# XiaRho/MADM

Measured on AMD Instinct MI355X. Metric: UNet feature-extract images/sec @512x512 bs=2/GPU, higher is better.
Workload: dtype f16; 1 GPU; configs[1]: SD-v1-4 VAE-encode + UNet single-timestep feature extractor (taps 5,8,11 'after'), 2x3x512x512 per GPU, t=0, LoRA off (shipped configs), seeded synthetic weights; global_batch=2, parallelism=replicas x1 (no collectives)

## Files before the change

madm_amd/csrc/conv3x3.hip:

```cpp
#include "conv3x3_common.hpp"

namespace {

template <typename T, int BN, bool FUSE, int NWS>
__global__ __launch_bounds__(256, (NWS == 2 || BN == 64) ? 2 : 1) void conv3x3_halo_kernel(const IgemmP p, const PatchDecode pd) {
    kernarg_touch<5>();
    constexpr int EPC = TT<T>::EPC;
    constexpr int BKE = 8 * EPC;
    constexpr int MI = 4, NI = BN / 32;
    constexpr int RB = BN / 32;
    constexpr int HI = (HPIX * 8 + 255) / 256;
    constexpr int HALO_U4 = HPIX * 8, W_U4 = BN * 8;
    constexpr unsigned OOB = 0x80000000u;
    extern __shared__ __attribute__((aligned(16))) char smem_raw[];
    u32x4* halo = reinterpret_cast<u32x4*>(smem_raw);
    u32x4* wlds = halo + 2 * HALO_U4;
    float2* gstat = reinterpret_cast<float2*>(wlds + 2 * W_U4);

    const int tid = threadIdx.x, lane = tid & 63, wave = tid >> 6;
    const int wm = wave >> 1, wn = wave & 1;
    const int cpos = tid & 7, lrow = tid >> 3;
    const int frow = lane & 15, fg = lane >> 4;
    const int z = blockIdx.z;

// ... 175 lines not shown
        }                                                                                           \
        C3_PRIO(0);                                                                                 \
        C3_PIN();                                                                                   \
        C3_STAMP(s_, 1);                                                                            \
        if ((s_) + 1 < S) C3_STORE_W((CUR) ^ 1, RS_);                                               \
        if (tap == 8 && next_chunk_) C3_STORE_HALO(((ck - ck0) + 1) & 1, ck + 1);                   \
        C3_STAMP(s_, 2);                                                                            \
        __syncthreads();                                                                            \
        C3_STAMP(s_, 3);                                                                            \
        if (++tap == 9) { tap = 0; ++ck; }                                                          \
    }
    int s = 0;
    if constexpr (NWS == 2) {
        for (; s + 1 < S; s += 2) {
            C3_STEP(s, 0, rw[0], rw[1]);
            C3_STEP(s + 1, 1, rw[1], rw[0]);
        }
        if (s < S) C3_STEP(s, 0, rw[0], rw[1]);
    } else {
        for (; s + NWS <= S; s += NWS) {
#pragma unroll
            for (int u = 0; u < NWS; ++u) C3_STEP(s + u, u & 1, rw[u], rw[(u + 1) % NWS]);
        }
#pragma unroll
        for (int u = 0; u < NWS - 1; ++u)
            if (s + u < S) C3_STEP(s + u, u & 1, rw[u], rw[(u + 1) % NWS]);
    }
#undef C3_STEP
#undef C3_LOAD_W
#undef C3_STORE_W
#undef C3_LOAD_HALO
#undef C3_STORE_HALO

    halo_tile_epilogue<T, BN>(p, acc, b, py0, px0, n0, z, reinterpret_cast<float*>(smem_raw));
}

template <typename T, int BN, bool FUSE, int NWS>
int launch_one(const IgemmP& p0, hipStream_t s) {
    IgemmP p = p0;
    constexpr size_t lds = (size_t)(2 * HPIX * 8 + 2 * BN * 8) * 16 + 32 * sizeof(float2);
    auto kern = conv3x3_halo_kernel<T, BN, FUSE, NWS>;
    static std::atomic<uint64_t> attr_done{0};
    if (int e = madm_raise_dynamic_lds(reinterpret_cast<const void*>(kern), (size_t)(lds), attr_done, "conv3x3")) return e;
    const int patchesX = (p.OW + TW - 1) / TW, patchesY = (p.OH + TH - 1) / TH;
    p.tilesN = (p.N + BN - 1) / BN;
    dim3 grid((unsigned)(p.B * patchesX * patchesY * p.tilesN), 1, (unsigned)p.splitk);
    PatchDecode pd;
    if (!patch_decode_fill(pd, patchesX, patchesY, p.tilesN, (long long)grid.x)) {
        madm_set_error("conv3x3: grid of %u blocks too large for the reciprocal patch decode", grid.x);
        return MADM_ERR_INVALID_ARG;
    }
    kern<<<grid, 256, lds, s>>>(p, pd);
    return madm_check_launch("conv3x3_halo_kernel");
}

}

template <typename T>
int launch_conv3x3_halo(const IgemmP& p, int bn, hipStream_t s) {
    const bool fuse = p.gn_sums1 != nullptr;
    if (bn == 128) return fuse ? launch_one<T, 128, true, 2>(p, s) : launch_one<T, 128, false, 2>(p, s);
    return fuse ? launch_one<T, 64, true, 2>(p, s) : launch_one<T, 64, false, 2>(p, s);
}
#ifdef C3_STAMPS
extern "C" int madm_debug_read_c3_stamps(unsigned long long* host, int n) {
    return (int)hipMemcpyFromSymbol(host, HIP_SYMBOL(g_c3_stamps), sizeof(unsigned long long) * n);
}
// ... 5 lines not shown
```

madm_amd/csrc/conv3x3_common.hpp:

```cpp
#pragma once
#include "igemm_common.hpp"

struct PatchDecode {
    int patchesX, patchesPerImg;
    unsigned m_tilesN, m_ppi, m_px;
};
__host__ inline unsigned patch_magic(unsigned d) { return d <= 1 ? 0u : (unsigned)((0x100000000ull + d - 1) / d); }
__host__ inline bool patch_decode_fill(PatchDecode& pd, int patchesX, int patchesY, int tilesN, long long blocks) {
    pd.patchesX = patchesX; pd.patchesPerImg = patchesX * patchesY;
    pd.m_tilesN = patch_magic((unsigned)tilesN); pd.m_ppi = patch_magic((unsigned)pd.patchesPerImg);
    pd.m_px = patch_magic((unsigned)patchesX);
    const unsigned long long lim = 0x100000000ull;
    return (unsigned long long)blocks * (unsigned)tilesN < lim && (unsigned long long)blocks * (unsigned)pd.patchesPerImg < lim &&
           (unsigned long long)pd.patchesPerImg * (unsigned)patchesX < lim;
}
__device__ __forceinline__ int magic_div(int x, unsigned m) { return m ? (int)__umulhi((unsigned)x, m) : x; }

namespace {

constexpr int TH = 8, TW = 16, HWD = TW + 2, HPIX = (TH + 2) * HWD;
#ifdef C3_STAMPS
__device__ unsigned long long g_c3_stamps[2048];
#endif

template <typename T, int EPC>
__device__ __forceinline__ u32x4 gn_act_chunk(u32x4 raw, const float* sc, const float* sh, int act) {
    float f[EPC];
    chunk_to_f32<T>(__builtin_bit_cast(uint4, raw), f);
#pragma unroll
    for (int j = 0; j < EPC; ++j) f[j] = f[j] * sc[j] + sh[j];
    act_inplace<EPC>(f, act);
    return __builtin_bit_cast(u32x4, f32_to_chunk<T>(f));
}

template <typename T, int BN>
__device__ __forceinline__ void halo_tile_epilogue(const IgemmP& p, f32x4 (&acc)[4][BN / 32], int b, int py0, int px0,
                                                   int n0, int z, float* red) {
    constexpr int MI = 4, NI = BN / 32;
    const int tid = threadIdx.x, lane = tid & 63, wave = tid >> 6;
    const int wm = wave >> 1, wn = wave & 1;
    const int frow = lane & 15, fg = lane >> 4;
    const bool want_stats = p.stats != nullptr && p.splitk == 1;
    const int nb = n0 + wn * (BN / 2) + fg * 4;
    f32x4 cs[NI], cq[NI], add[NI];
#pragma unroll
    for (int j = 0; j < NI; ++j) { cs[j] = f32x4{0.f, 0.f, 0.f, 0.f}; cq[j] = f32x4{0.f, 0.f, 0.f, 0.f}; }
    if (p.splitk == 1) epilogue_consts<NI>(p, nb, b, add);
    int mrow[MI];
#pragma unroll
    for (int i = 0; i < MI; ++i) {
        const int oy = py0 + wm * 4 + i, ox = px0 + frow;
        mrow[i] = (oy < p.OH && ox < p.OW) ? (b * p.OH + oy) * p.OW + ox : -1;
    }
    if (p.splitk > 1) {
#pragma unroll
        for (int i = 0; i < MI; ++i) {
            if (mrow[i] < 0) continue;
#pragma unroll
            for (int j = 0; j < NI; ++j) {
                const f32x4 v = acc[i][j];
                if (nb + 16 * j < p.N)
                    *reinterpret_cast<float4*>(p.ws + ((size_t)z * p.M + mrow[i]) * p.N + nb + 16 * j) =
                        make_float4(v[0], v[1], v[2], v[3]);
            }
        }
    } else {
        epilogue_tile<T, MI, NI>(p, mrow, nb, add, false, acc);
        if (want_stats) {
#pragma unroll
            for (int i = 0; i < MI; ++i) {
                if (mrow[i] < 0) continue;
#pragma unroll
                for (int j = 0; j < NI; ++j)
                    if (nb + 16 * j < p.N) { cs[j] += acc[i][j]; cq[j] += acc[i][j] * acc[i][j]; }
            }
        }
    }
    if (want_stats) {
#pragma unroll
        for (int j = 0; j < NI; ++j) {
#pragma unroll
            for (int r = 0; r < 4; ++r) {
                cs[j][r] = row16_sum(cs[j][r]);
                cq[j][r] = row16_sum(cq[j][r]);
            }
            if (frow == 0) {
                float* dst = red + ((wm * BN) + wn * (BN / 2) + j * 16 + fg * 4) * 2;
#pragma unroll
                for (int r = 0; r < 4; ++r) { dst[2 * r] = cs[j][r]; dst[2 * r + 1] = cq[j][r]; }
            }
        }
    }
    if (want_stats) {
        __syncthreads();
        for (int c = tid; c < 2 * BN; c += 256) {
            const int n = n0 + (c >> 1);
            if (n < p.N)
                atomicAdd(p.stats + ((size_t)b * p.N + n0) * 2 + c, (double)red[c] + (double)red[2 * BN + c]);
        }
    }
}

}
```

madm_amd/csrc/conv3x3_dma.hip:

```cpp
#include "conv3x3_common.hpp"

namespace {

#if defined(__HIP_DEVICE_COMPILE__)
template <int N> __device__ __forceinline__ void c3_wait_vmcnt() { asm volatile("s_waitcnt vmcnt(%0)" ::"n"(N) : "memory"); }
template <int N> __device__ __forceinline__ void c3_wait_lgkmcnt() { asm volatile("s_waitcnt lgkmcnt(%0)" ::"n"(N) : "memory"); }
#endif

#ifdef C3D_STAMPS
__device__ unsigned long long g_c3d_stamps[256];
#define C3D_STAMP(k_) if (blockIdx.x == 5 && blockIdx.z == 0 && threadIdx.x == 0 && (k_) < 256) g_c3d_stamps[(k_)] = __builtin_readcyclecounter();
#else
#define C3D_STAMP(k_)
#endif

template <typename T, int BN, bool FUSE>
__global__ __launch_bounds__(256, 2) void conv3x3_halo_dma_kernel(const IgemmP p, const PatchDecode pd) {
    C3D_STAMP(0);
    kernarg_touch<5>();
#if defined(__HIP_DEVICE_COMPILE__)
    constexpr int EPC = TT<T>::EPC;
    constexpr int BKE = 8 * EPC;
    constexpr int MI = 4, NI = BN / 32;
    constexpr int LW = BN / 32;
// ... 180 lines not shown
                for (int i = 0; i < MI; ++i)
                    asm volatile("ds_read_b128 %0, %1" : "=v"(af[1][i]) : "v"(ah[(r_ + i) * 3 + sx_] ^ 64u));
#pragma unroll
                for (int j = 0; j < NI; ++j)
                    asm volatile("ds_read_b128 %0, %1 offset:%2" : "=v"(wf[1][j]) : "v"(wf1), "n"(cur * kW_BYTES + j * 2048));
                c3_wait_lgkmcnt<MI + NI>();
                __builtin_amdgcn_sched_barrier(0);
#pragma unroll
                for (int i = 0; i < MI; ++i)
#pragma unroll
                    for (int j = 0; j < NI; ++j)
                        mma16<T>(__builtin_bit_cast(uint4, wf[0][j]), __builtin_bit_cast(uint4, af[0][i]), acc[i][j]);
                c3_wait_lgkmcnt<0>();
                __builtin_amdgcn_sched_barrier(0);
#pragma unroll
                for (int i = 0; i < MI; ++i)
#pragma unroll
                    for (int j = 0; j < NI; ++j)
                        mma16<T>(__builtin_bit_cast(uint4, wf[1][j]), __builtin_bit_cast(uint4, af[1][i]), acc[i][j]);
            }
            __builtin_amdgcn_sched_barrier(0);
            if (tap == 8 && next_chunk) {
                __builtin_amdgcn_s_barrier();
                D3_STORE_HALO(ck + 1);
            }
        }
    }
#undef D3_LOAD_HALO
#undef D3_STORE_HALO
#undef D3_DMA_W
    C3D_STAMP(4);
    c3_wait_vmcnt<0>();
    __syncthreads();
    halo_tile_epilogue<T, BN>(p, acc, b, py0, px0, n0, z, reinterpret_cast<float*>(smem_raw));
    C3D_STAMP(5);
#ifdef C3D_STAMPS
    asm volatile("s_waitcnt vmcnt(0)" ::: "memory");
    C3D_STAMP(6);
#endif
#endif
}

template <typename T, int BN, bool FUSE>
int launch_dma_one(const IgemmP& p0, hipStream_t s) {
    IgemmP p = p0;
    constexpr size_t lds = (size_t)(HPIX * 8 + 3 * BN * 8) * 16 + 32 * sizeof(float2);
    auto kern = conv3x3_halo_dma_kernel<T, BN, FUSE>;
    static std::atomic<uint64_t> attr_done{0};
    if (int e = madm_raise_dynamic_lds(reinterpret_cast<const void*>(kern), (size_t)(lds), attr_done, "conv3x3 (LDS-DMA)")) return e;
    const int patchesX = (p.OW + TW - 1) / TW, patchesY = (p.OH + TH - 1) / TH;
    p.tilesN = (p.N + BN - 1) / BN;
    dim3 grid((unsigned)(p.B * patchesX * patchesY * p.tilesN), 1, (unsigned)p.splitk);
    PatchDecode pd;
    if (!patch_decode_fill(pd, patchesX, patchesY, p.tilesN, (long long)grid.x)) {
        madm_set_error("conv3x3 (LDS-DMA): grid of %u blocks too large for the reciprocal patch decode", grid.x);
        return MADM_ERR_INVALID_ARG;
    }
    kern<<<grid, 256, lds, s>>>(p, pd);
    return madm_check_launch("conv3x3_halo_dma_kernel");
}

}

template <typename T>
int launch_conv3x3_halo_dma(const IgemmP& p, int bn, hipStream_t s) {
    const bool fuse = p.gn_sums1 != nullptr;
    if (bn == 128) return fuse ? launch_dma_one<T, 128, true>(p, s) : launch_dma_one<T, 128, false>(p, s);
// ... 11 lines not shown
```

madm_amd/csrc/igemm.hip:

```cpp
#include <algorithm>
#include <cstdio>
#include <cstdlib>
#include <vector>
#include <atomic>
#include "igemm_common.hpp"

namespace {
#ifdef GLDS_STAMPS
__device__ unsigned long long g_reg_stamps[64];
#define REG_BSTAMP(k_) if (blockIdx.x == 7 && blockIdx.z == 0 && threadIdx.x == 0) g_reg_stamps[(k_)] = __builtin_readcyclecounter();
#else
#define REG_BSTAMP(k_)
#endif

template <int BM, int BN>
__device__ __forceinline__ bool cstash_request(const IgemmP& p, int m0, int n0, u32x4& cb, u32x4& cr, u32x4& cl) {
    constexpr unsigned OOB = 0x80000000u;
    const int tid = threadIdx.x;
    const bool on = p.splitk == 1 && tid < BN / 4;
    const unsigned nbytes = (unsigned)p.N * 4u;
    const float* rowp = nullptr;
    if (p.rowvec) {
        const int OHW = p.OH * p.OW;
        int mlast = m0 + BM; if (mlast > p.M) mlast = p.M; mlast -= 1;
        const int img0 = m0 / OHW;
        if (mlast / OHW == img0) rowp = p.rowvec + (size_t)img0 * p.ldrv;
    }
    const float* dummy = reinterpret_cast<const float*>(p.w);
    const __amdgpu_buffer_rsrc_t rb = __builtin_amdgcn_make_buffer_rsrc((void*)(p.bias ? p.bias : dummy), 0, p.bias ? nbytes : 0u, 0x00020000);
    const __amdgpu_buffer_rsrc_t rr = __builtin_amdgcn_make_buffer_rsrc((void*)(rowp ? rowp : dummy), 0, rowp ? nbytes : 0u, 0x00020000);
    const __amdgpu_buffer_rsrc_t rl = __builtin_amdgcn_make_buffer_rsrc((void*)(p.ln_cs ? p.ln_cs : dummy), 0, p.ln_cs ? nbytes : 0u, 0x00020000);
    const unsigned off = on ? (unsigned)(n0 + tid * 4) * 4u : OOB;
    cb = __builtin_amdgcn_raw_buffer_load_b128(rb, off, 0, 0);
    cr = __builtin_amdgcn_raw_buffer_load_b128(rr, off, 0, 0);
    cl = __builtin_amdgcn_raw_buffer_load_b128(rl, off, 0, 0);
    return on;
}
template <int BN>
__device__ __forceinline__ void cstash_park(bool on, u32x4 cb_, u32x4 cr_, u32x4 cl_, float* cstash) {
    if (on) {
        const float4 cb = __builtin_bit_cast(float4, cb_), cr = __builtin_bit_cast(float4, cr_);
        *reinterpret_cast<float4*>(cstash + threadIdx.x * 4) = make_float4(cb.x + cr.x, cb.y + cr.y, cb.z + cr.z, cb.w + cr.w);
        *reinterpret_cast<float4*>(cstash + BN + threadIdx.x * 4) = __builtin_bit_cast(float4, cl_);
    }
}

template <typename T, int BM, int BN>
__device__ __forceinline__ void igemm_tile_epilogue(const IgemmP& p, f32x4 (&acc)[BM / 32][BN / 32], int m0, int n0,
                                                    int z, float* red, float (&lns)[BM / 32], float (&lnq)[BM / 32],
                                                    const float* cstash, const float* cstash_row, const float* cstash_ln) {
    constexpr int MI = BM / 32, NI = BN / 32;
    const int tid = threadIdx.x, lane = tid & 63, wave = tid >> 6;
    const int wm = wave >> 1, wn = wave & 1;
    const int frow = lane & 15, fg = lane >> 4;
    const int OHW = p.OH * p.OW;
    const bool want_stats = p.stats != nullptr && p.splitk == 1;
    int mlast = m0 + BM; if (mlast > p.M) mlast = p.M; mlast -= 1;
    const int img0 = m0 / OHW;
    const bool one_image = (mlast / OHW) == img0;
    const int nb = n0 + wn * (BN / 2) + fg * 4;
    f32x4 cs[NI], cq[NI], add[NI];
#pragma unroll
    for (int j = 0; j < NI; ++j) { cs[j] = f32x4{0.f, 0.f, 0.f, 0.f}; cq[j] = f32x4{0.f, 0.f, 0.f, 0.f}; }
    if (p.splitk == 1) {
#pragma unroll
        for (int j = 0; j < NI; ++j) {
            const float4 c = *reinterpret_cast<const float4*>(cstash + wn * (BN / 2) + fg * 4 + 16 * j);
            add[j] = f32x4{c.x, c.y, c.z, c.w};
            if (cstash_row) {
                const float4 r = *reinterpret_cast<const float4*>(cstash_row + wn * (BN / 2) + fg * 4 + 16 * j);
                add[j] += f32x4{r.x, r.y, r.z, r.w};
            }
        }
    }
    if (p.ln_cs) {
        f32x4 csv[NI];
#pragma unroll
        for (int j = 0; j < NI; ++j) {
            const float4 c = *reinterpret_cast<const float4*>(cstash_ln + wn * (BN / 2) + fg * 4 + 16 * j);
            csv[j] = f32x4{c.x, c.y, c.z, c.w};
        }
        const float inv_k = 1.0f / (float)p.K;
        float2* lx = reinterpret_cast<float2*>(red + 4 * BN);
#pragma unroll
        for (int i = 0; i < MI; ++i) {
            float sx = lns[i], sq = lnq[i];
            sx += __shfl_xor(sx, 16); sq += __shfl_xor(sq, 16);
            sx += __shfl_xor(sx, 32); sq += __shfl_xor(sq, 32);
            lns[i] = sx; lnq[i] = sq;
            if (fg == 0) lx[(wave * MI + i) * 16 + frow] = make_float2(sx, sq);
        }
        __syncthreads();
#pragma unroll
        for (int i = 0; i < MI; ++i) {
            const float2 o = lx[((wave ^ 1) * MI + i) * 16 + frow];
            const float sx = lns[i] + o.x, sq = lnq[i] + o.y;
            const float mean = sx * inv_k;
            float var = sq * inv_k - mean * mean;
            var = var < 0.f ? 0.f : var;
            const float rstd = 1.0f / sqrtf(var + p.ln_eps);
#pragma unroll
            for (int j = 0; j < NI; ++j) acc[i][j] = (acc[i][j] - mean * csv[j]) * rstd;
        }
    }
    REG_BSTAMP(8);
    int mrow[MI];
#pragma unroll
    for (int i = 0; i < MI; ++i) {
        const int m = m0 + wm * (BM / 2) + i * 16 + frow;
        mrow[i] = m < p.M ? m : -1;
    }
    if (p.splitk > 1) {
#pragma unroll
        for (int i = 0; i < MI; ++i) {
            if (mrow[i] < 0) continue;
#pragma unroll
            for (int j = 0; j < NI; ++j) {
                const f32x4 v = acc[i][j];
                if (nb + 16 * j < p.N)
                    *reinterpret_cast<float4*>(p.ws + ((size_t)z * p.M + mrow[i]) * p.N + nb + 16 * j) =
                        make_float4(v[0], v[1], v[2], v[3]);
            }
        }
    } else {
        epilogue_tile<T, MI, NI>(p, mrow, nb, add, !one_image, acc);
        if (want_stats) {
#pragma unroll
            for (int i = 0; i < MI; ++i) {
                if (mrow[i] < 0) continue;
#pragma unroll
                for (int j = 0; j < NI; ++j) {
                    if (nb + 16 * j >= p.N) continue;
                    if (one_image) { cs[j] += acc[i][j]; cq[j] += acc[i][j] * acc[i][j]; }
                    else stats_add_elementwise(p, mrow[i], nb + 16 * j, acc[i][j]);
                }
            }
        }
    }
    REG_BSTAMP(9 + MI);
    if (want_stats && one_image) {
#pragma unroll
        for (int j = 0; j < NI; ++j) {
#pragma unroll
            for (int r = 0; r < 4; ++r) {
                cs[j][r] = row16_sum(cs[j][r]);
                cq[j][r] = row16_sum(cq[j][r]);
            }
            if (frow == 0) {
                float* dst = red + ((wm * BN) + wn * (BN / 2) + j * 16 + fg * 4) * 2;
#pragma unroll
                for (int r = 0; r < 4; ++r) { dst[2 * r] = cs[j][r]; dst[2 * r + 1] = cq[j][r]; }
            }
        }
    }
    if (want_stats && one_image) {
        __syncthreads();
        for (int c = tid; c < 2 * BN; c += 256) {
            const int n = n0 + (c >> 1);
            if (n < p.N) atomicAdd(p.stats + ((size_t)img0 * p.N + n0) * 2 + c, (double)red[c] + (double)red[2 * BN + c]);
        }
    }
}

template <typename T, int BM, int BN, int NST, bool LIN>
__global__ __launch_bounds__(256, (BM * BN >= 128 * 128) ? 1 : 2) void igemm_kernel(const IgemmP p) {
    kernarg_touch<5>();
    constexpr int EPC = TT<T>::EPC;
    constexpr int BKE = 8 * EPC;
    constexpr int RA = BM / 32, RB = BN / 32;
    constexpr int MI = BM / 32, NI = BN / 32;
    __shared__ __attribute__((aligned(16))) uint4 smem[2 * (BM + BN) * 8];
    __shared__ __attribute__((aligned(16))) float cstash[2 * BN];

    const int tid = threadIdx.x, lane = tid & 63, wave = tid >> 6;
    REG_BSTAMP(0);
    const int wm = wave >> 1, wn = wave & 1;
    int bid = blockIdx.x;
    {
        const int nb = gridDim.x, q = nb >> 3, r = nb & 7, x = bid & 7, i = bid >> 3;
        bid = (x < r ? x * (q + 1) : r * (q + 1) + (x - r) * q) + i;
    }
    const int tn = bid % p.tilesN, tm = bid / p.tilesN;
    const int m0 = tm * BM, n0 = tn * BN;
    const int z = blockIdx.z;
    const int chunk = tid & 7, lrow = tid >> 3;
// ... 115 lines not shown
            uint4 af[MI], wf[NI];                                                                   \
            _Pragma("unroll") for (int i = 0; i < MI; ++i)                                          \
                af[i] = sA[(wm * (BM / 2) + i * 16 + frow) * 8 + c];                                \
            _Pragma("unroll") for (int j = 0; j < NI; ++j)                                          \
                wf[j] = sB[(wn * (BN / 2) + j * 16 + frow) * 8 + c];                                \
            _Pragma("unroll") for (int i = 0; i < MI; ++i)                                          \
                _Pragma("unroll") for (int j = 0; j < NI; ++j) mma16<T>(wf[j], af[i], acc[i][j]);   \
            if (ln_on && kk == wn) {    \
                _Pragma("unroll") for (int i = 0; i < MI; ++i) ln_accum<T>(af[i], lns[i], lnq[i]);  \
            }                                                                                       \
        }                                                                                           \
    }
    REG_BSTAMP(2);
    for (int kt = kt0; kt < kt1; kt += NST) {
#pragma unroll
        for (int u = 0; u < NST; ++u) {
            const int t = kt + u;
            if (t < kt1) {
                const int cur = (t - kt0) & 1;
                if (t + NST < kt1) IGEMM_LOAD_TILE(t + NST, ra[u], rb[u]);
                __builtin_amdgcn_sched_barrier(0);
                IGEMM_COMPUTE(cur);
                __builtin_amdgcn_sched_barrier(0);
                if (t + 1 < kt1) IGEMM_STORE_TILE(cur ^ 1, ra[(u + 1) % NST], rb[(u + 1) % NST]);
                __syncthreads();
            }
        }
    }
#undef IGEMM_COMPUTE
#undef IGEMM_LOAD_TILE
#undef IGEMM_STORE_TILE

    REG_BSTAMP(3);
    igemm_tile_epilogue<T, BM, BN>(p, acc, m0, n0, z, reinterpret_cast<float*>(smem), lns, lnq, cstash, nullptr, cstash + BN);
    REG_BSTAMP(4);
#ifdef GLDS_STAMPS
    asm volatile("s_waitcnt vmcnt(0)" ::: "memory");
    REG_BSTAMP(5);
#endif
}

#define GLDS_ASM(...) asm volatile(__VA_ARGS__)
#ifdef GLDS_STAMPS
__device__ unsigned long long g_glds_stamps[2048];
#endif
#if defined(__HIP_DEVICE_COMPILE__)
template <int N> __device__ __forceinline__ void wait_vmcnt() { GLDS_ASM("s_waitcnt vmcnt(%0)" ::"n"(N) : "memory"); }
template <int N> __device__ __forceinline__ void wait_lgkmcnt() { GLDS_ASM("s_waitcnt lgkmcnt(%0)" ::"n"(N) : "memory"); }
#endif

template <typename T, int BM, int BN, int NS, bool LIN>
__global__ __launch_bounds__(256, BM * BN >= 128 * 128 ? (NS == 2 ? 2 : 1) : (NS == 3 && BM == 64 ? 3 : 2)) void igemm_glds_kernel(const IgemmP p) {
#if defined(__HIP_DEVICE_COMPILE__)
    kernarg_touch<5>();
    constexpr int EPC = TT<T>::EPC;
    constexpr int BKE = 8 * EPC;
    constexpr int MI = BM / 32, NI = BN / 32;
    constexpr int ROWS = BM + BN;
    constexpr int LPT = ROWS / 32;
    constexpr int TILE_U4 = ROWS * 8;
    static_assert(NS >= 2 && NS <= 4 && ROWS % 32 == 0, "ring depth / tile shape");
    extern __shared__ __attribute__((aligned(16))) uint4 gsmem[];
    __shared__ __attribute__((aligned(16))) float cstash[3 * 256];
    typedef __attribute__((address_space(3))) char lds_char;

    const int tid = threadIdx.x, lane = tid & 63;
    const int wave = __builtin_amdgcn_readfirstlane(tid >> 6);
    const int wm = wave >> 1, wn = wave & 1;
#ifdef GLDS_STAMPS
#define GLDS_BSTAMP(k_) if (blockIdx.x == 0 && blockIdx.z == 0 && tid == 0) g_glds_stamps[2000 + (k_)] = __builtin_readcyclecounter();
#else
#define GLDS_BSTAMP(k_)
#endif
    GLDS_BSTAMP(0);
    int bid = blockIdx.x;
    {
        const int nb = gridDim.x, q = nb >> 3, r = nb & 7, x = bid & 7, i = bid >> 3;
        bid = (x < r ? x * (q + 1) : r * (q + 1) + (x - r) * q) + i;
    }
    const int tn = bid % p.tilesN, tm = bid / p.tilesN;
    const int m0 = tm * BM, n0 = tn * BN;
    const int z = blockIdx.z;
    const int rsub = lane >> 3, cpos = lane & 7;

    constexpr unsigned OOB = 0x80000000u;
    const int OHW = p.OH * p.OW;
    int a_b[LPT], a_iy[LPT], a_ix[LPT];
    unsigned wvoff[LPT], swz[LPT];
#pragma unroll
    for (int i = 0; i < LPT; ++i) {
        const int row = (wave * LPT + i) * 8 + rsub;
        swz[i] = (unsigned)((cpos ^ (row & 7)) * EPC);
        a_b[i] = 0; a_iy[i] = -(1 << 24); a_ix[i] = 0; wvoff[i] = OOB;
        if (row < BM) {
// ... 149 lines not shown
            _Pragma("unroll") for (int i = 0; i < MI; ++i)                                                       \
                _Pragma("unroll") for (int j = 0; j < NI; ++j)                                                   \
                    mma16<T>(__builtin_bit_cast(uint4, wf[0][j]), __builtin_bit_cast(uint4, af[0][i]), acc[i][j]); \
            wait_lgkmcnt<0>();                                                                                   \
            __builtin_amdgcn_sched_barrier(0);                                                                   \
            _Pragma("unroll") for (int i = 0; i < MI; ++i)                                                       \
                _Pragma("unroll") for (int j = 0; j < NI; ++j)                                                   \
                    mma16<T>(__builtin_bit_cast(uint4, wf[1][j]), __builtin_bit_cast(uint4, af[1][i]), acc[i][j]); \
            if (ln_on) {                 \
                if (wn == 0) {                                                                                   \
                    _Pragma("unroll") for (int i = 0; i < MI; ++i)                                               \
                        ln_accum<T>(__builtin_bit_cast(uint4, af[0][i]), lns[i], lnq[i]);                        \
                } else {                                                                                         \
                    _Pragma("unroll") for (int i = 0; i < MI; ++i)                                               \
                        ln_accum<T>(__builtin_bit_cast(uint4, af[1][i]), lns[i], lnq[i]);                        \
                }                                                                                                \
            }                                                                                                    \
        }                                                                                                        \
        __builtin_amdgcn_sched_barrier(0);                                                                       \
        GLDS_STAMP(t, 3);                                                                                        \
    }
    int t = 0;
    for (; t + NS <= nt; t += NS) {
#pragma unroll
        for (int u = 0; u < NS; ++u) GLDS_STEP(t + u, u, (u + NS - 1) % NS);
    }
#pragma unroll
    for (int u = 0; u < NS - 1; ++u)
        if (t + u < nt) GLDS_STEP(t + u, u, (u + NS - 1) % NS);
#undef GLDS_STEP
#undef GLDS_LOAD_TILE
    GLDS_BSTAMP(3);
    __syncthreads();
    igemm_tile_epilogue<T, BM, BN>(p, acc, m0, n0, z, reinterpret_cast<float*>(gsmem), lns, lnq, cstash, cstash + 256, cstash + 512);
    GLDS_BSTAMP(4);
#endif
}

template <typename T>
__global__ __launch_bounds__(256) void splitk_reduce_kernel(const IgemmP p) {
    __shared__ float red[16][64][2];
    const int tx = threadIdx.x & 15, ty = threadIdx.x >> 4;
    const int n = (blockIdx.x * 16 + tx) * 4;
    const int mbase = blockIdx.y * 16;
    const int OHW = p.OH * p.OW;
    int mlast = mbase + 16; if (mlast > p.M) mlast = p.M; mlast -= 1;
    const int img0 = mbase / OHW;
    const bool one_image = (mlast / OHW) == img0;
    const bool want_stats = p.stats != nullptr;
    f32x4 v = f32x4{0.f, 0.f, 0.f, 0.f};
    const int m = mbase + ty;
    const bool valid = m < p.M && n < p.N;
    if (valid) {
        const bool plain = p.epilogue != MADM_EPI_GEGLU;
        f32x4 add = f32x4{0.f, 0.f, 0.f, 0.f}, res = f32x4{0.f, 0.f, 0.f, 0.f};
        if (plain) {
            if (p.bias) {
                const float4 b = *reinterpret_cast<const float4*>(p.bias + n);
                add = f32x4{b.x, b.y, b.z, b.w};
            }
            if (p.rowvec) {
                const float4 r = *reinterpret_cast<const float4*>(p.rowvec + (size_t)(m / OHW) * p.ldrv + n);
                add[0] += r.x; add[1] += r.y; add[2] += r.z; add[3] += r.w;
            }
            if (p.residual) res = load4<T>(reinterpret_cast<const T*>(p.residual) + (size_t)m * p.ldr + n);
        }
        const float* src = p.ws + (size_t)m * p.N + n;
// ... 316 lines not shown
        MADM_REQUIRE(a->KH == 1 && a->KW == 1 && a->stride == 1 && a->pad_t == 0 && a->pad_l == 0 && !a->upsample &&
                     a->C2 == 0 && a->OH == a->IH && a->OW == a->IW,
                     "conv2d: the folded LayerNorm needs a linear layer / 1x1 conv over ONE source (K = C1)");
        MADM_REQUIRE(!a->gn_sums1 && a->ln_eps > 0.f && a->splitk == 1,
                     "conv2d: folded LayerNorm: no fused GroupNorm, eps > 0, splitk == 1 (every block must see whole rows)");
    }
    MADM_REQUIRE(!a->stats || a->epilogue != MADM_EPI_GEGLU, "conv2d: fused statistics cannot follow GEGLU");
    p.C1 = a->C1; p.C2 = a->C2; p.Ctot = a->C1 + a->C2;
    p.B = a->B; p.IH = a->IH; p.IW = a->IW; p.OH = a->OH; p.OW = a->OW;
    p.KH = a->KH; p.KW = a->KW; p.stride = a->stride; p.pad_t = a->pad_t; p.pad_l = a->pad_l;
    p.upsample = a->upsample ? 1 : 0;
    p.N = a->N; p.K = r.K; p.M = r.M;
    MADM_REQUIRE(!a->rowvec || (a->ldrv >= a->N && a->ldrv % 4 == 0), "conv2d: bad ldrv=%d", a->ldrv);
    p.ldr = a->ldr; p.ldo = a->ldo; p.ldrv = a->ldrv; p.epilogue = a->epilogue;
    p.ldw = a->ldw ? a->ldw : p.K;
    p.out_f32 = a->out_f32 ? 1 : 0;
    MADM_REQUIRE(p.ldw >= p.K && p.ldw % (bke / 8) == 0, "conv2d: bad weight row stride ldw=%d", p.ldw);
    MADM_REQUIRE(!p.out_f32 || (a->epilogue != MADM_EPI_GEGLU && !a->residual), "conv2d: out_f32 cannot follow GEGLU / residual");
    p.ld1 = a->ld1 ? a->ld1 : a->C1;
    p.ld2 = a->ld2 ? a->ld2 : a->C2;
    MADM_REQUIRE(p.ld1 >= a->C1 && p.ld2 >= a->C2 && p.ld1 % (bke / 8) == 0 && p.ld2 % (bke / 8) == 0,
                 "conv2d: bad source row strides ld1=%d ld2=%d", p.ld1, p.ld2);
    {
        const size_t es = madm_esize(a->dtype);
        const size_t px = (size_t)a->B * a->IH * a->IW;
        const size_t b1 = ((px - 1) * p.ld1 + a->C1) * es;
        const size_t b2 = a->C2 ? ((px - 1) * p.ld2 + a->C2) * es : 0;
        const size_t bw = ((size_t)(a->N - 1) * p.ldw + p.K) * es;
        MADM_REQUIRE(b1 < 0x80000000ull && b2 < 0x80000000ull && bw < 0x80000000ull,
                     "conv2d: tensors must stay below 2 GiB (32-bit buffer offsets)");
        p.bytes1 = (unsigned)b1; p.bytes2 = (unsigned)b2; p.bytesw = (unsigned)bw;
    }
    p.nk = r.k_steps();
    MADM_REQUIRE((long long)p.nk * (std::min(a->splitk, p.nk) + 1) < 0x7fffffffLL, "conv2d: K too large for the 32-bit slice arithmetic");
    return MADM_OK;
}

template <typename T, int BM, int BN, int NS, bool LIN>
int launch_glds_v(const IgemmP& p, dim3 grid, hipStream_t s) {
    constexpr size_t lds = (size_t)NS * (BM + BN) * 128;
    auto kern = igemm_glds_kernel<T, BM, BN, NS, LIN>;
    static std::atomic<uint64_t> attr_done{0};
    if (int e = madm_raise_dynamic_lds(reinterpret_cast<const void*>(kern), (size_t)(lds), attr_done, "igemm (LDS-DMA)")) return e;
    kern<<<grid, 256, lds, s>>>(p);
    return madm_check_launch("igemm_glds_kernel");
}

template <typename T, int BM, int BN, int NS>
int launch_glds(const IgemmP& p, dim3 grid, hipStream_t s, bool lin) {
    return lin ? launch_glds_v<T, BM, BN, NS, true>(p, grid, s) : launch_glds_v<T, BM, BN, NS, false>(p, grid, s);
}

template <typename T>
int launch(const IgemmP& p0, int t, hipStream_t s, const PostGn& pn) {
    IgemmP p = p0;
    const Tile& ti = *tile_info(t);
    const int bm = ti.bm, bn = ti.bn;
    int rc;
    if (ti.family == APANEL) return launch_igemm_apanel<T>(p, s);
    if (ti.family == H16) rc = launch_conv3x3_h16<T>(p, bn, s);
    else if (ti.family == HALO_DMA) rc = launch_conv3x3_halo_dma<T>(p, bn, s);
    else if (ti.family == HALO) rc = launch_conv3x3_halo<T>(p, bn, s);
    else {
        p.tilesN = (p.N + bn - 1) / bn;
        const int tilesM = (p.M + bm - 1) / bm;
        dim3 grid((unsigned)(tilesM * p.tilesN), 1, (unsigned)p.splitk);
        const bool lin = p.KH == 1 && p.KW == 1 && p.stride == 1 && p.pad_t == 0 && p.pad_l == 0 && !p.upsample &&
                         p.OH == p.IH && p.OW == p.IW;
        if (t == 1) igemm_kernel<T, 128, 128, 2, false><<<grid, 256, 0, s>>>(p);
        else if (t == 2 && lin) igemm_kernel<T, 128, 64, 3, true><<<grid, 256, 0, s>>>(p);
        else if (t == 2) igemm_kernel<T, 128, 64, 3, false><<<grid, 256, 0, s>>>(p);
        else if (t == 6) igemm_kernel<T, 64, 64, 8, false><<<grid, 256, 0, s>>>(p);
        else if (t == 7) { if (int e = launch_glds<T, 64, 64, 4>(p, grid, s, lin)) return e; }
        else if (t == 8) { if (int e = launch_glds<T, 128, 64, 3>(p, grid, s, lin)) return e; }
        else if (t == 11) { if (int e = launch_glds<T, 64, 64, 3>(p, grid, s, lin)) return e; }
        else if (t == 14) { if (int e = launch_glds<T, 128, 128, 3>(p, grid, s, lin)) return e; }
        else if (t == 15) { if (int e = launch_glds<T, 128, 128, 2>(p, grid, s, lin)) return e; }
        else if (t == 16) { if (int e = launch_glds<T, 64, 64, 2>(p, grid, s, lin)) return e; }
        else if (t == 17) { if (int e = launch_glds<T, 128, 64, 2>(p, grid, s, lin)) return e; }
        else if (lin) igemm_kernel<T, 64, 64, 4, true><<<grid, 256, 0, s>>>(p);
        else igemm_kernel<T, 64, 64, 4, false><<<grid, 256, 0, s>>>(p);
        rc = madm_check_launch("igemm_kernel");
    }
    if (rc) return rc;
    if (p.splitk > 1 && pn.gamma) {
        const size_t lds = post_gn_lds(p.OH * p.OW, p.N, pn.G);
        const dim3 pgrid((unsigned)pn.G, (unsigned)p.B);
        if ((p.N / pn.G) % 4 == 0) {
            auto kern = splitk_groupnorm_kernel<T, 4>;
            static std::atomic<uint64_t> attr_done{0};
            if (int e = madm_raise_dynamic_lds(reinterpret_cast<const void*>(kern), PGN_MAX_LDS, attr_done, "split-K + GroupNorm")) return e;
// ... 109 lines not shown
```

madm_amd/csrc/igemm_common.hpp:

```cpp
#pragma once
#include "common.hpp"

typedef unsigned int u32x4 __attribute__((ext_vector_type(4)));

struct IgemmP {
    const char* in1; const char* in2; const char* w;
    const float* bias; const float* rowvec; const char* residual; char* out; float* ws; double* stats;
    int C1, C2, Ctot, B, IH, IW, OH, OW, KH, KW, stride, pad_t, pad_l, upsample;
    int N, K, M, ldr, ldo, ldrv, epilogue, splitk, tilesN, nk, ld1, ld2, ldw, out_f32;
    unsigned bytes1, bytes2, bytesw;
    const double* gn_sums1; const double* gn_sums2; const float* gn_gamma; const float* gn_beta;
    int gn_G; float gn_eps; unsigned gn_magic; int act;
    const float* ln_cs; float ln_eps;
};

template <typename T> __device__ __forceinline__ void ln_accum(const uint4& a, float& s, float& q);
template <> __device__ __forceinline__ void ln_accum<float>(const uint4& a, float& s, float& q) {
    const float4 v = __builtin_bit_cast(float4, a);
    s += (v.x + v.y) + (v.z + v.w);
    q = fmaf(v.x, v.x, q); q = fmaf(v.y, v.y, q); q = fmaf(v.z, v.z, q); q = fmaf(v.w, v.w, q);
}
template <> __device__ __forceinline__ void ln_accum<f16_t>(const uint4& a, float& s, float& q) {
    typedef _Float16 h2 __attribute__((ext_vector_type(2)));
    const h2 one = {(_Float16)1.0f, (_Float16)1.0f};
    const unsigned w[4] = {a.x, a.y, a.z, a.w};
#pragma unroll
    for (int i = 0; i < 4; ++i) {
        const h2 v = __builtin_bit_cast(h2, w[i]);
        s = __builtin_amdgcn_fdot2(v, one, s, false);
        q = __builtin_amdgcn_fdot2(v, v, q, false);
    }
}
template <> __device__ __forceinline__ void ln_accum<bf16_t>(const uint4& a, float& s, float& q) {
    typedef __bf16 b2 __attribute__((ext_vector_type(2)));
    const b2 one = {(__bf16)1.0f, (__bf16)1.0f};
    const unsigned w[4] = {a.x, a.y, a.z, a.w};
#pragma unroll
    for (int i = 0; i < 4; ++i) {
        const b2 v = __builtin_bit_cast(b2, w[i]);
        s = __builtin_amdgcn_fdot2_f32_bf16(v, one, s, false);
        q = __builtin_amdgcn_fdot2_f32_bf16(v, v, q, false);
    }
}

__device__ __forceinline__ void gn_fold_groups(const IgemmP& p, int b, float2* gstat) {
    const int G = p.gn_G, cpg = p.Ctot / G, C2 = p.Ctot - p.C1;
// ... 214 lines not shown
            for (int j = 0; j < NI; ++j) r[i][j] = load4<T>(rp + (nb + 16 * j < p.N ? nb + 16 * j : p.N - 4));
        }
#pragma unroll
        for (int i = 0; i < MI; ++i)
#pragma unroll
            for (int j = 0; j < NI; ++j) acc[i][j] += r[i][j];
    }
    if (p.epilogue == MADM_EPI_RELU) {
#pragma unroll
        for (int i = 0; i < MI; ++i)
#pragma unroll
            for (int j = 0; j < NI; ++j) {
                f32x4& v = acc[i][j];
                v[0] = fmaxf(v[0], 0.f); v[1] = fmaxf(v[1], 0.f); v[2] = fmaxf(v[2], 0.f); v[3] = fmaxf(v[3], 0.f);
            }
    }
#pragma unroll
    for (int i = 0; i < MI; ++i) {
        if (mrow[i] < 0) continue;
        if (p.out_f32) {
            float* op = reinterpret_cast<float*>(p.out) + (size_t)mrow[i] * p.ldo + nb;
#pragma unroll
            for (int j = 0; j < NI; ++j)
                if (nb + 16 * j < p.N) store4<float>(op + 16 * j, acc[i][j]);
        } else {
            T* op = reinterpret_cast<T*>(p.out) + (size_t)mrow[i] * p.ldo + nb;
#pragma unroll
            for (int j = 0; j < NI; ++j)
                if (nb + 16 * j < p.N) store4<T>(op + 16 * j, acc[i][j]);
        }
    }
}

__device__ __forceinline__ void stats_add_elementwise(const IgemmP& p, int m, int n, f32x4 v) {
    const int bi = m / (p.OH * p.OW);
    double* s = p.stats + ((size_t)bi * p.N + n) * 2;
#pragma unroll
    for (int r = 0; r < 4; ++r) {
        atomicAdd(s + 2 * r, (double)v[r]);
        atomicAdd(s + 2 * r + 1, (double)(v[r] * v[r]));
    }
}


template <typename T> int launch_conv3x3_halo(const IgemmP& p, int bn, hipStream_t s);
template <typename T> int launch_conv3x3_halo_dma(const IgemmP& p, int bn, hipStream_t s);
template <typename T> int launch_igemm_apanel(const IgemmP& p, hipStream_t s);
int igemm_apanel_bm(int K, int esize);
template <typename T> int launch_conv3x3_h16(const IgemmP& p, int bn, hipStream_t s);
```

Before: 378.6 images/s.

## Stage f16 GEMM/conv epilogue through LDS for wide 16-byte stores and residual DMA

Adds a 'wide' epilogue path for f16 GLDS and halo-DMA conv kernels. The output tile is staged in LDS (reusing the halo and ring buffers), then written to global memory with coalesced 16-byte stores. Residual inputs are prefetched into LDS with buffer_load_lds DMA instead of being read per fragment. This targets the narrow, scattered 8-byte stores and loads of the fragment-layout epilogue, at the cost of extra barriers, LDS traffic and host-side eligibility checks on alignment.

```diff
diff --git a/madm_amd/csrc/conv3x3.hip b/madm_amd/csrc/conv3x3.hip
--- a/madm_amd/csrc/conv3x3.hip
+++ b/madm_amd/csrc/conv3x3.hip
@@ -231,7 +231,7 @@
 #undef C3_LOAD_HALO
 #undef C3_STORE_HALO
 
-    halo_tile_epilogue<T, BN>(p, acc, b, py0, px0, n0, z, reinterpret_cast<float*>(smem_raw));
+    halo_tile_epilogue<T, BN>(p, acc, b, py0, px0, n0, z, reinterpret_cast<float*>(smem_raw), false, 0);
 }
 
 template <typename T, int BN, bool FUSE, int NWS>
diff --git a/madm_amd/csrc/conv3x3_common.hpp b/madm_amd/csrc/conv3x3_common.hpp
--- a/madm_amd/csrc/conv3x3_common.hpp
+++ b/madm_amd/csrc/conv3x3_common.hpp
@@ -35,13 +35,24 @@
 
 template <typename T, int BN>
 __device__ __forceinline__ void halo_tile_epilogue(const IgemmP& p, f32x4 (&acc)[4][BN / 32], int b, int py0, int px0,
-                                                   int n0, int z, float* red) {
+                                                   int n0, int z, float* red, const bool wide_ok, const int lds_bytes) {
     constexpr int MI = 4, NI = BN / 32;
     const int tid = threadIdx.x, lane = tid & 63, wave = tid >> 6;
     const int wm = wave >> 1, wn = wave & 1;
     const int frow = lane & 15, fg = lane >> 4;
     const bool want_stats = p.stats != nullptr && p.splitk == 1;
     const int nb = n0 + wn * (BN / 2) + fg * 4;
+    const bool wide = sizeof(T) == 2 && wide_ok && p.wide;
+    char* const tile = reinterpret_cast<char*>(red) + WIDE_TILE_OFS;
+    const bool rshared = wide_tile_bytes<T, TH * TW, BN>() + TH * TW * BN * (int)sizeof(T) > lds_bytes;
+    char* const rtile = rshared ? tile : reinterpret_cast<char*>(red) + wide_tile_bytes<T, TH * TW, BN>();
+    auto row_of = [&](int r) {
+        const int oy = py0 + (r >> 4), ox = px0 + (r & 15);
+        return (oy < p.OH && ox < p.OW) ? (b * p.OH + oy) * p.OW + ox : -1;
+    };
+    if constexpr (sizeof(T) == 2) {
+        if (wide && p.residual) wide_residual_dma<T, TH * TW, BN>(p, rtile, n0, row_of);
+    }
     f32x4 cs[NI], cq[NI], add[NI];
 #pragma unroll
     for (int j = 0; j < NI; ++j) { cs[j] = f32x4{0.f, 0.f, 0.f, 0.f}; cq[j] = f32x4{0.f, 0.f, 0.f, 0.f}; }
@@ -65,7 +76,11 @@
             }
         }
     } else {
-        epilogue_tile<T, MI, NI>(p, mrow, nb, add, false, acc);
+        if (wide) {
+            if constexpr (sizeof(T) == 2) wide_tile_write<T, MI, NI>(p, add, acc, tile, rtile, rshared);
+        } else {
+            epilogue_tile<T, MI, NI>(p, mrow, nb, add, false, acc);
+        }
         if (want_stats) {
 #pragma unroll
             for (int i = 0; i < MI; ++i) {
@@ -91,6 +106,21 @@
             }
         }
     }
+    if constexpr (sizeof(T) == 2) {
+        if (wide) {
+            __syncthreads();
+            const bool full = py0 + TH <= p.OH && px0 + TW <= p.OW && n0 + BN <= p.N;
+            wide_tile_store<T, TH * TW, BN>(p, tile, n0, full, row_of);
+            if (want_stats) {
+                for (int c = tid; c < 2 * BN; c += 256) {
+                    const int n = n0 + (c >> 1);
+                    if (n < p.N)
+                        atomicAdd(p.stats + ((size_t)b * p.N + n0) * 2 + c, (double)red[c] + (double)red[2 * BN + c]);
+                }
+            }
+            return;
+        }
+    }
     if (want_stats) {
         __syncthreads();
         for (int c = tid; c < 2 * BN; c += 256) {
diff --git a/madm_amd/csrc/conv3x3_dma.hip b/madm_amd/csrc/conv3x3_dma.hip
--- a/madm_amd/csrc/conv3x3_dma.hip
+++ b/madm_amd/csrc/conv3x3_dma.hip
@@ -236,7 +236,8 @@
     C3D_STAMP(4);
     c3_wait_vmcnt<0>();
     __syncthreads();
-    halo_tile_epilogue<T, BN>(p, acc, b, py0, px0, n0, z, reinterpret_cast<float*>(smem_raw));
+    static_assert(wide_tile_bytes<bf16_t, TH * TW, BN>() <= (HALO_U4 + 3 * W_U4) * 16, "wide epilogue: the output tile reuses halo + ring");
+    halo_tile_epilogue<T, BN>(p, acc, b, py0, px0, n0, z, reinterpret_cast<float*>(smem_raw), true, (HALO_U4 + 3 * W_U4) * 16);
     C3D_STAMP(5);
 #ifdef C3D_STAMPS
     asm volatile("s_waitcnt vmcnt(0)" ::: "memory");
diff --git a/madm_amd/csrc/igemm.hip b/madm_amd/csrc/igemm.hip
--- a/madm_amd/csrc/igemm.hip
+++ b/madm_amd/csrc/igemm.hip
@@ -48,7 +48,8 @@
 template <typename T, int BM, int BN>
 __device__ __forceinline__ void igemm_tile_epilogue(const IgemmP& p, f32x4 (&acc)[BM / 32][BN / 32], int m0, int n0,
                                                     int z, float* red, float (&lns)[BM / 32], float (&lnq)[BM / 32],
-                                                    const float* cstash, const float* cstash_row, const float* cstash_ln) {
+                                                    const float* cstash, const float* cstash_row, const float* cstash_ln, const bool wide_ok,
+                                                    const int lds_bytes) {
     constexpr int MI = BM / 32, NI = BN / 32;
     const int tid = threadIdx.x, lane = tid & 63, wave = tid >> 6;
     const int wm = wave >> 1, wn = wave & 1;
@@ -59,6 +60,14 @@
     const int img0 = m0 / OHW;
     const bool one_image = (mlast / OHW) == img0;
     const int nb = n0 + wn * (BN / 2) + fg * 4;
+    const bool wide = sizeof(T) == 2 && wide_ok && p.wide && !(p.rowvec && !one_image);
+    char* const tile = reinterpret_cast<char*>(red) + WIDE_TILE_OFS;
+    const bool rshared = wide_tile_bytes<T, BM, BN>() + BM * BN * (int)sizeof(T) > lds_bytes;
+    char* const rtile = rshared ? tile : reinterpret_cast<char*>(red) + wide_tile_bytes<T, BM, BN>();
+    if constexpr (sizeof(T) == 2) {
+        if (wide && p.residual) wide_residual_dma<T, BM, BN>(p, rtile, n0, [&](int r) { return m0 + r < p.M ? m0 + r : -1; });
+    }
+    static_assert(16 * BN + 512 * MI <= WIDE_TILE_OFS, "wide epilogue: the tile must not overlap red / lx");
     f32x4 cs[NI], cq[NI], add[NI];
 #pragma unroll
     for (int j = 0; j < NI; ++j) { cs[j] = f32x4{0.f, 0.f, 0.f, 0.f}; cq[j] = f32x4{0.f, 0.f, 0.f, 0.f}; }
@@ -123,7 +132,11 @@
             }
         }
     } else {
-        epilogue_tile<T, MI, NI>(p, mrow, nb, add, !one_image, acc);
+        if (wide) {
+            if constexpr (sizeof(T) == 2) wide_tile_write<T, MI, NI>(p, add, acc, tile, rtile, rshared);
+        } else {
+            epilogue_tile<T, MI, NI>(p, mrow, nb, add, !one_image, acc);
+        }
         if (want_stats) {
 #pragma unroll
             for (int i = 0; i < MI; ++i) {
@@ -151,6 +164,20 @@
 #pragma unroll
                 for (int r = 0; r < 4; ++r) { dst[2 * r] = cs[j][r]; dst[2 * r + 1] = cq[j][r]; }
             }
+        }
+    }
+    if constexpr (sizeof(T) == 2) {
+        if (wide) {
+            __syncthreads();
+            const bool full = m0 + BM <= p.M && n0 + BN <= p.N;
+            wide_tile_store<T, BM, BN>(p, tile, n0, full, [&](int r) { return m0 + r < p.M ? m0 + r : -1; });
+            if (want_stats && one_image) {
+                for (int c = tid; c < 2 * BN; c += 256) {
+                    const int n = n0 + (c >> 1);
+                    if (n < p.N) atomicAdd(p.stats + ((size_t)img0 * p.N + n0) * 2 + c, (double)red[c] + (double)red[2 * BN + c]);
+                }
+            }
+            return;
         }
     }
     if (want_stats && one_image) {
@@ -332,7 +359,7 @@
 #undef IGEMM_STORE_TILE
 
     REG_BSTAMP(3);
-    igemm_tile_epilogue<T, BM, BN>(p, acc, m0, n0, z, reinterpret_cast<float*>(smem), lns, lnq, cstash, nullptr, cstash + BN);
+    igemm_tile_epilogue<T, BM, BN>(p, acc, m0, n0, z, reinterpret_cast<float*>(smem), lns, lnq, cstash, nullptr, cstash + BN, false, 0);
     REG_BSTAMP(4);
 #ifdef GLDS_STAMPS
     asm volatile("s_waitcnt vmcnt(0)" ::: "memory");
@@ -360,6 +387,8 @@
     constexpr int LPT = ROWS / 32;
     constexpr int TILE_U4 = ROWS * 8;
     static_assert(NS >= 2 && NS <= 4 && ROWS % 32 == 0, "ring depth / tile shape");
+    static_assert(wide_tile_bytes<bf16_t, BM, BN>() <= NS * TILE_U4 * 16, "wide epilogue: the output tile reuses the ring");
+    constexpr bool WIDE_OK = !(BM * BN >= 128 * 128 && NS == 3);
     extern __shared__ __attribute__((aligned(16))) uint4 gsmem[];
     __shared__ __attribute__((aligned(16))) float cstash[3 * 256];
     typedef __attribute__((address_space(3))) char lds_char;
@@ -575,7 +604,7 @@
 #undef GLDS_LOAD_TILE
     GLDS_BSTAMP(3);
     __syncthreads();
-    igemm_tile_epilogue<T, BM, BN>(p, acc, m0, n0, z, reinterpret_cast<float*>(gsmem), lns, lnq, cstash, cstash + 256, cstash + 512);
+    igemm_tile_epilogue<T, BM, BN>(p, acc, m0, n0, z, reinterpret_cast<float*>(gsmem), lns, lnq, cstash, cstash + 256, cstash + 512, WIDE_OK, NS * TILE_U4 * 16);
     GLDS_BSTAMP(4);
 #endif
 }
@@ -958,6 +987,7 @@
         p.bytes1 = (unsigned)b1; p.bytes2 = (unsigned)b2; p.bytesw = (unsigned)bw;
     }
     p.nk = r.k_steps();
+    p.wide = 0;
     MADM_REQUIRE((long long)p.nk * (std::min(a->splitk, p.nk) + 1) < 0x7fffffffLL, "conv2d: K too large for the 32-bit slice arithmetic");
     return MADM_OK;
 }
@@ -983,6 +1013,7 @@
     const Tile& ti = *tile_info(t);
     const int bm = ti.bm, bn = ti.bn;
     int rc;
+    p.wide = (ti.family == GLDS || ti.family == HALO_DMA) && wide_epilogue_ok(p, sizeof(T)) ? 1 : 0;
     if (ti.family == APANEL) return launch_igemm_apanel<T>(p, s);
     if (ti.family == H16) rc = launch_conv3x3_h16<T>(p, bn, s);
     else if (ti.family == HALO_DMA) rc = launch_conv3x3_halo_dma<T>(p, bn, s);
diff --git a/madm_amd/csrc/igemm_common.hpp b/madm_amd/csrc/igemm_common.hpp
--- a/madm_amd/csrc/igemm_common.hpp
+++ b/madm_amd/csrc/igemm_common.hpp
@@ -12,6 +12,7 @@
     const double* gn_sums1; const double* gn_sums2; const float* gn_gamma; const float* gn_beta;
     int gn_G; float gn_eps; unsigned gn_magic; int act;
     const float* ln_cs; float ln_eps;
+    int wide;
 };
 
 template <typename T> __device__ __forceinline__ void ln_accum(const uint4& a, float& s, float& q);
@@ -292,6 +293,165 @@
     }
 }
 
+constexpr int WIDE_TILE_OFS = 4096;
+template <typename T, int ROWS, int BN> constexpr int wide_tile_bytes() { return WIDE_TILE_OFS + ROWS * (BN * (int)sizeof(T) + 16); }
+
+inline bool wide_epilogue_ok(const IgemmP& p, size_t esize) {
+    const int ocols = p.epilogue == MADM_EPI_GEGLU ? p.N / 2 : p.N;
+    if (p.residual && (p.ldr % 8 != 0 || (reinterpret_cast<size_t>(p.residual) & 15) != 0 ||
+                       (size_t)p.M * (size_t)p.ldr * esize >= 0x80000000ull))
+        return false;
+    return esize == 2 && p.splitk == 1 && !p.out_f32 && ocols % 8 == 0 && p.ldo % 8 == 0 &&
+           (reinterpret_cast<size_t>(p.out) & 15) == 0;
+}
+
+__device__ __forceinline__ int wide_tid() {
+    int t = (int)threadIdx.x;
+    asm volatile("" : "+v"(t));
+    return t;
+}
+
+template <int CPR> constexpr int wide_swz_shift() { return CPR >= 16 ? 0 : (CPR == 8 ? 1 : 2); }
+
+template <typename T, int ROWS, int COLS, typename RowOf>
+__device__ __forceinline__ void wide_residual_dma_cols(const IgemmP& p, char* rtile, int c0, int ncols, RowOf row_of) {
+#if defined(__HIP_DEVICE_COMPILE__)
+    typedef __attribute__((address_space(3))) char lds_char;
+    constexpr int CPR = COLS * (int)sizeof(T) / 16, RPI = 64 / CPR, PIECES = ROWS / RPI / 4, EPP = 16 / (int)sizeof(T);
+    constexpr int SH = wide_swz_shift<CPR>();
+    static_assert(CPR >= 4 && CPR <= 16 && ROWS % (RPI * 4) == 0, "residual DMA: 1 KB pieces, four waves");
+    const __amdgpu_buffer_rsrc_t rsr = __builtin_amdgcn_make_buffer_rsrc(
+        (void*)p.residual, 0, (unsigned)((size_t)p.M * (size_t)p.ldr * sizeof(T)), 0x00020000);
+    const int tid = wide_tid(), lane = tid & 63;
+    const int wave = __builtin_amdgcn_readfirstlane(tid >> 6);
+#pragma unroll
+    for (int t = 0; t < PIECES; ++t) {
+        const int q = wave * PIECES + t;
+        const int r = q * RPI + lane / CPR, pos = lane % CPR;
+        const int c = pos ^ ((r >> SH) & (CPR - 1));
+        const int m = row_of(r), n = c0 + c * EPP;
+        const unsigned off = (m >= 0 && n < ncols) ? (unsigned)(((size_t)m * p.ldr + n) * sizeof(T)) : 0x80000000u;
+        __builtin_amdgcn_raw_ptr_buffer_load_lds(rsr, (lds_char*)rtile + q * 1024, 16, off, 0, 0, 0);
+    }
+#endif
+}
+template <typename T, int ROWS, int BN, typename RowOf>
+__device__ __forceinline__ void wide_residual_dma(const IgemmP& p, char* rtile, int n0, RowOf row_of) {
+    if (p.epilogue == MADM_EPI_GEGLU) wide_residual_dma_cols<T, ROWS, BN / 2>(p, rtile, n0 >> 1, p.N >> 1, row_of);
+    else wide_residual_dma_cols<T, ROWS, BN>(p, rtile, n0, p.N, row_of);
+}
+
+template <typename T, int MI, int NI>
+__device__ __forceinline__ void wide_tile_write(const IgemmP& p, const f32x4 (&add)[NI], f32x4 (&acc)[MI][NI], char* tile,
+                                                const char* rtile, const bool rshared) {
+    constexpr int BN = NI * 32;
+    const int tid = wide_tid();
+    const int lane = tid & 63, wave = tid >> 6;
+    const int wm = wave >> 1, wn = wave & 1, frow = lane & 15, fg = lane >> 4;
+    if (p.residual) {
+#if defined(__HIP_DEVICE_COMPILE__)
+        asm volatile("s_waitcnt vmcnt(0)" ::: "memory");
+#endif
+        __syncthreads();
+    }
+    if (p.epilogue == MADM_EPI_GEGLU) {
+        constexpr int ROW = (BN / 2) * (int)sizeof(T) + 16;
+        constexpr int RB = (BN / 2) * (int)sizeof(T), CPR = RB / 16, SH = wide_swz_shift<CPR>();
+#pragma unroll
+        for (int i = 0; i < MI; ++i)
+#pragma unroll
+            for (int j = 0; j < NI; ++j) {
+                const f32x4 t = acc[i][j] + add[j];
+                acc[i][j] = f32x4{t[0] * gelu_erf_f(t[1]), t[2] * gelu_erf_f(t[3]), 0.f, 0.f};
+            }
+        if (p.residual) {
+#pragma unroll
+            for (int i = 0; i < MI; ++i) {
+                const int r = (wm * MI + i) * 16 + frow;
+#pragma unroll
+                for (int j = 0; j < NI; ++j) {
+                    const int byte = (wn * (BN / 4) + fg * 2 + 8 * j) * (int)sizeof(T);
+                    const T* rp = reinterpret_cast<const T*>(rtile + r * RB + (((byte >> 4) ^ ((r >> SH) & (CPR - 1))) << 4) + (byte & 15));
+                    acc[i][j][0] += TT<T>::ld(rp);
+                    acc[i][j][1] += TT<T>::ld(rp + 1);
+                }
+            }
+            if (rshared) __syncthreads();
+        }
+#pragma unroll
+        for (int i = 0; i < MI; ++i) {
+            char* row = tile + ((wm * MI + i) * 16 + frow) * ROW + (wn * (BN / 4) + fg * 2) * (int)sizeof(T);
+#pragma unroll
+            for (int j = 0; j < NI; ++j) store2<T>(reinterpret_cast<T*>(row + j * 8 * (int)sizeof(T)), acc[i][j][0], acc[i][j][1]);
+        }
+        return;
+    }
+    constexpr int ROW = BN * (int)sizeof(T) + 16;
+#pragma unroll
+    for (int i = 0; i < MI; ++i)
+#pragma unroll
+        for (int j = 0; j < NI; ++j) acc[i][j] += add[j];
+    if (p.residual) {
+        constexpr int RB = BN * (int)sizeof(T), CPR = RB / 16, SH = wide_swz_shift<CPR>();
+#pragma unroll
+        for (int i = 0; i < MI; ++i) {
+            const int r = (wm * MI + i) * 16 + frow;
+#pragma unroll
+            for (int j = 0; j < NI; ++j) {
+                const int byte = (wn * (BN / 2) + fg * 4 + 16 * j) * (int)sizeof(T);
+                acc[i][j] += load4<T>(reinterpret_cast<const T*>(rtile + r * RB + (((byte >> 4) ^ ((r >> SH) & (CPR - 1))) << 4) + (byte & 15)));
+            }
+        }
+        if (rshared) __syncthreads();
+    }
+    if (p.epilogue == MADM_EPI_RELU) {
+#pragma unroll
+        for (int i = 0; i < MI; ++i)
+#pragma unroll
+            for (int j = 0; j < NI; ++j) {
+                f32x4& v = acc[i][j];
+                v[0] = fmaxf(v[0], 0.f); v[1] = fmaxf(v[1], 0.f); v[2] = fmaxf(v[2], 0.f); v[3] = fmaxf(v[3], 0.f);
+            }
+    }
+#pragma unroll
+    for (int i = 0; i < MI; ++i) {
+        char* row = tile + ((wm * MI + i) * 16 + frow) * ROW + (wn * (BN / 2) + fg * 4) * (int)sizeof(T);
+#pragma unroll
+        for (int j = 0; j < NI; ++j) store4<T>(reinterpret_cast<T*>(row + j * 16 * (int)sizeof(T)), acc[i][j]);
+    }
+}
+
+template <typename T, int ROWS, int COLS, typename RowOf>
+__device__ __forceinline__ void wide_tile_store_cols(const IgemmP& p, const char* tile, int c0, int ncols, bool full, RowOf row_of) {
+    constexpr int ROW = COLS * (int)sizeof(T) + 16, CPR = COLS * (int)sizeof(T) / 16, EPP = 16 / (int)sizeof(T);
+    static_assert((ROWS * CPR) % 256 == 0, "wide epilogue: whole rounds of 256 pieces");
+    T* out = reinterpret_cast<T*>(p.out);
+    const int tid = wide_tid();
+    if (full) {
+#pragma unroll
+        for (int c = 0; c < ROWS * CPR; c += 256) {
+            const int q = c + tid, r = q / CPR, ch = q % CPR;
+            const uint4 v = *reinterpret_cast<const uint4*>(tile + r * ROW + ch * 16);
+            *reinterpret_cast<uint4*>(out + (size_t)row_of(r) * p.ldo + c0 + ch * EPP) = v;
+        }
+        return;
+    }
+#pragma unroll
+    for (int c = 0; c < ROWS * CPR; c += 256) {
+        const int q = c + tid, r = q / CPR, ch = q % CPR;
+        const int m = row_of(r), n = c0 + ch * EPP;
+        if (m >= 0 && n < ncols) {
+            const uint4 v = *reinterpret_cast<const uint4*>(tile + r * ROW + ch * 16);
+            *reinterpret_cast<uint4*>(out + (size_t)m * p.ldo + n) = v;
+        }
+    }
+}
+template <typename T, int ROWS, int BN, typename RowOf>
+__device__ __forceinline__ void wide_tile_store(const IgemmP& p, const char* tile, int n0, bool full, RowOf row_of) {
+    if (p.epilogue == MADM_EPI_GEGLU) wide_tile_store_cols<T, ROWS, BN / 2>(p, tile, n0 >> 1, p.N >> 1, full, row_of);
+    else wide_tile_store_cols<T, ROWS, BN>(p, tile, n0, p.N, full, row_of);
+}
+
 __device__ __forceinline__ void stats_add_elementwise(const IgemmP& p, int m, int n, f32x4 v) {
     const int bi = m / (p.OH * p.OW);
     double* s = p.stats + ((size_t)bi * p.N + n) * 2;
```

Result: no change. 382.4 images/s, median of 6 (+1.0%).
